# CederGroupHub/chgnet

Hardware: AMD Instinct MI355X
Metric: structures/s (energy+force+stress) on batched ~50-atom crystals (higher is better)
Workload: dtype f32; 1 GPU; 1024 x LiMnO2 5x1x1 (40 atoms, sigma=0.01 frac perturbation) per GPU, task efs; structures_per_gpu=1024, atoms=40960, directed_bonds=3535504, angles=4125764, bond_graph_nodes=213755, weights=random-init 0.3.0 architecture (tests/golden/weights_seed0.npz), parallelism=structures sharded over 1 GPU(s), RCCL all-gather of energies only, process_group_ranks=1, energies_in_all_gather=1024, comm=none (single rank)

## Files before the change

chgnet_amd/csrc/kernels_angle_w.h:

```cpp
#pragma once

#include "blk_shape.h"
#include "kernels_conv.h"

namespace chg {

constexpr int TS64 = D + PAD;
constexpr int TILE64_FLOATS = TILE_ROWS * TS64;
constexpr int WIN_LIST = 32;
constexpr int WIN_MAX_GRID = 1024;
constexpr int WIN_MIN_ATOMS_PER_WAVE = 3;

struct WinIndex {
  int* flag;
  int *wave_head, *next_atom;
  int* xatom;
  int *na, *boff, *aoff;
  int* toff;
  int* toff4;
  int *head, *rank;
  int* list;
  int *q_a, *q_ctr, *q_b1c, *q_b2c, *q_ab1, *q_ab2;
  int* abbond;
  int4* rows;
// ... 116 lines not shown
  }
  w.xatom[i] = lo;
}

__device__ __forceinline__ unsigned wave_min_u32(unsigned v) {
#define CHG_DPP_MIN(ctrl) v = min(v, (unsigned)__builtin_amdgcn_update_dpp((int)v, (int)v, (ctrl), 0xF, 0xF, false))
  CHG_DPP_MIN(0xB1);
  CHG_DPP_MIN(0x4E);
  CHG_DPP_MIN(0x141);
  CHG_DPP_MIN(0x140);
#undef CHG_DPP_MIN
  const auto r = __builtin_amdgcn_permlane16_swap(v, v, false, false);
  const unsigned s = min((unsigned)r[0], (unsigned)r[1]);
  const auto q = __builtin_amdgcn_permlane32_swap(s, s, false, false);
  return min((unsigned)q[0], (unsigned)q[1]);
}

static __global__ __launch_bounds__(64) void k_win_schedule(int grid, WinIndex w) {
  const int gi = blockIdx.x, lane = threadIdx.x;
  const int spx = grid >> 6;
  const int x = gi / spx, sub = gi - x * spx;
  const int head_slot = ((((sub << 3) + (lane / WAVES)) << 3) + x) * WAVES + (lane % WAVES);
  if (w.flag[0] != 1) { w.wave_head[head_slot] = -1; return; }
  const int c0 = w.xatom[gi], c1 = w.xatom[gi + 1];
  unsigned load = 0;
  int head = -1, tail = -1;
  for (int cb = c0; cb < c1; cb += 64) {
    const int nn = w.na[min(cb + lane, c1 - 1)];
    const int m = min(64, c1 - cb);
    for (int i = 0; i < m; ++i) {
      const int n = __builtin_amdgcn_readlane(nn, i);
      if (n < 2) continue;
      const unsigned cost = (unsigned)(n * (n - 1) + TILE_ROWS - 1) / TILE_ROWS + 1;
      const unsigned best = wave_min_u32((load << 6) | (unsigned)lane);
      if ((int)(best & 63u) == lane) {
        const int c = cb + i;
        load += cost;
        w.next_atom[c] = -1;
        if (tail < 0) head = c; else w.next_atom[tail] = c;
        tail = c;
      }
    }
  }
  w.wave_head[head_slot] = head;
}

static __global__ void k_win_atoms(int N, WinIndex w) {
  const int c = blockIdx.x * blockDim.x + threadIdx.x;
  if (c < N) w.atoms[c] = make_int4(w.na[c], w.aoff[c], w.boff[c], w.next_atom[c]);
}

struct AngleWArgs {
  AngleArgs a;
  WinIndex w;
  int n_atoms;
};

struct AngleBwdWArgs {
  const int* flag;
  const float* image;
  const float* w_ang;
  GatedW gw;
  const float *R, *S, *ang, *wbgc, *Gagg, *zsave;
  float *Gang, *GR, *GS, *Gwbgc;
  int first_gang;
  const int4* rows;
  const int* abbond;
  const int4* atoms;
  const int* wave_head;
  const int *toff, *na, *aoff, *boff, *q_a, *q_b1c, *q_b2c, *q_ab2;
  int n_atoms;
};
inline AngleBwdWArgs angle_bwd_w_args(const AngleArgs& a, const WinIndex& w, int n_atoms) {
  AngleBwdWArgs k{};
  k.flag = w.flag; k.image = a.image; k.w_ang = a.w_ang; k.gw = a.gw;
  k.R = a.R; k.S = a.S; k.ang = a.ang; k.wbgc = a.wbgc; k.Gagg = a.Gagg; k.zsave = a.zsave;
  k.Gang = a.Gang; k.GR = a.GR; k.GS = a.GS; k.Gwbgc = a.Gwbgc; k.first_gang = a.first_gang;
  k.rows = w.rows; k.abbond = w.abbond; k.atoms = w.atoms; k.wave_head = w.wave_head;
  k.toff = w.toff; k.na = w.na; k.aoff = w.aoff; k.boff = w.boff; k.q_a = w.q_a; k.q_b1c = w.q_b1c; k.q_b2c = w.q_b2c; k.q_ab2 = w.q_ab2;
  k.n_atoms = n_atoms;
  return k;
}

template <class T, bool A32 = false>
__device__ __forceinline__ T index_load(const T* __restrict__ base, int i) {
  if constexpr (A32) return *reinterpret_cast<const T*>(reinterpret_cast<const char*>(base) + (unsigned)i * (unsigned)sizeof(T));
  else return base[i];
}
__device__ __forceinline__ int4 index_load_uniform(const int4* base, int i) {
#if defined(__HIP_DEVICE_COMPILE__)
  typedef const int __attribute__((address_space(4))) * ConstInt;
  ConstInt q = (ConstInt)(unsigned long long)(base + i);
  return make_int4(q[0], q[1], q[2], q[3]);
#else
  return base[i];
#endif
}

template <bool HIDDEN> constexpr int win_ns() { return HIDDEN ? 13 : 14; }
template <bool HIDDEN> constexpr int win_pst() { return 2 * D; }
constexpr size_t WIN_RM_ANG = rm_image_bytes(2 * D, D), WIN_RM_W2 = rm_image_bytes(D, D);

template <bool HIDDEN>
constexpr size_t angle_w_lds() {
  const size_t weights = HIDDEN ? WIN_RM_ANG + 2 * WIN_RM_W2 : 16 * (size_t)(2 * IMG128);
  return weights + sizeof(float) * (VEC_SLOTS * D + WAVES * TILE64_FLOATS + WAVES * win_ns<HIDDEN>() * win_pst<HIDDEN>());
}

struct Gather64 { f32x4 a[TILE_ROWS / 4], b[TILE_ROWS / 4], c[TILE_ROWS / 4]; };
template <bool A32 = false>
__device__ __forceinline__ void gather64_issue(Gather64& gr, const float* __restrict__ t0, int i0, int ld0, const float* __restrict__ t1, int i1,
                                               int ld1, const float* __restrict__ t2, int i2, int ld2, int lane, int c0 = 0, int c1 = 0, int c2 = 0) {
  const int sub = lane >> 4, t = lane & 15;
  int r0[TILE_ROWS / 4], r1[TILE_ROWS / 4], r2[TILE_ROWS / 4];
#pragma unroll
  for (int it = 0; it < TILE_ROWS / 4; ++it) {
    const int rr = 4 * it + sub;
    r0[it] = __shfl(i0, rr); r1[it] = __shfl(i1, rr); r2[it] = __shfl(i2, rr);
  }
#pragma unroll
  for (int it = 0; it < TILE_ROWS / 4; ++it) {
    gr.a[it] = *grow<f32x4, A32>(t0, (unsigned)r0[it], ld0, c0 + 4 * t);
    gr.b[it] = *grow<f32x4, A32>(t1, (unsigned)r1[it], ld1, c1 + 4 * t);
    gr.c[it] = *grow<f32x4, A32>(t2, (unsigned)r2[it], ld2, c2 + 4 * t);
  }
}
__device__ __forceinline__ void gather64_commit(const Gather64& gr, float* tile, int lane) {
  const int sub = lane >> 4, t = lane & 15;
#pragma unroll
  for (int it = 0; it < TILE_ROWS / 4; ++it)
    *reinterpret_cast<f32x4*>(tile + (4 * it + sub) * TS64 + 4 * t) = (gr.a[it] + gr.b[it]) + gr.c[it];
}

struct Cols64 { float v[TILE_ROWS]; };
__device__ __forceinline__ void to_columns(const V64& x, float* T, float* Trow, int g, int lane, Cols64& c) {
  write_dl<VT>(Trow, g, x.t);
  __builtin_amdgcn_wave_barrier();
#pragma unroll
  for (int rr = 0; rr < TILE_ROWS; ++rr) c.v[rr] = T[rr * TS64 + lane];
  __builtin_amdgcn_wave_barrier();
}
__device__ __forceinline__ int fresh_uniform(int v) {
  asm volatile("" : "+s"(v));
  return v;
}
__device__ __forceinline__ unsigned run_starts64(int key, int cur, int nvalid, int lane) {
  const int prev = __builtin_amdgcn_update_dpp(cur, key, 0x111 , 0xF, 0xF, false);
  return (unsigned)__builtin_amdgcn_ballot_w64(key != prev && lane < nvalid);
}
template <int NB, bool A32 = false>
__device__ __forceinline__ void run_sum64(const Cols64 (&c)[NB], int nvalid, int key, unsigned starts, float (&sum)[NB], int& cur, float* __restrict__ dst,
                                          int ld, int col) {
  nvalid = fresh_uniform(nvalid);
#pragma unroll
  for (int rr = 0; rr < TILE_ROWS; ++rr) {
    if (rr < nvalid) {
      if (starts & (1u << rr)) {
        if (cur >= 0) {
          float* d = grow<float, A32>(dst, (unsigned)cur, ld, col);
#pragma unroll
          for (int q = 0; q < NB; ++q) atomicAdd(d + q * D, sum[q]);
        }
#pragma unroll
        for (int q = 0; q < NB; ++q) sum[q] = 0.f;
        cur = __builtin_amdgcn_readlane(key, rr);
      }
#pragma unroll
      for (int q = 0; q < NB; ++q) sum[q] += c[q].v[rr];
    }
  }
}
template <int NB, bool A32 = false>
__device__ __forceinline__ void run_flush64(float (&sum)[NB], int& cur, float* __restrict__ dst, int ld, int col) {
  if (cur >= 0) {
    float* d = grow<float, A32>(dst, (unsigned)cur, ld, col);
#pragma unroll
    for (int q = 0; q < NB; ++q) atomicAdd(d + q * D, sum[q]);
  }
#pragma unroll
  for (int q = 0; q < NB; ++q) sum[q] = 0.f;
  cur = -1;
}
template <bool A32 = false>
__device__ __forceinline__ void row_add64(const Cols64& c, int nvalid, float* __restrict__ base, int row, int ld, int lane) {
  nvalid = fresh_uniform(nvalid);
#pragma unroll
  for (int rr = 0; rr < TILE_ROWS; ++rr)
    if (rr < nvalid) atomicAdd(grow<float, A32>(base, (unsigned)__builtin_amdgcn_readlane(row, rr), ld, lane), c.v[rr]);
}
template <int NB>
__device__ __forceinline__ void private_add(const Cols64 (&c)[NB], int nvalid, int slot, float* pacc, float* dump, int lane) {
  nvalid = fresh_uniform(nvalid);
#pragma unroll
  for (int rr = 0; rr < TILE_ROWS; rr += 2) {
    const int sa = __builtin_amdgcn_readlane(slot, rr), sb = __builtin_amdgcn_readlane(slot, rr + 1);
    float* pa = (rr < nvalid && sa >= 0) ? pacc + sa * (NB * D) : dump;
    float* pb = (rr + 1 < nvalid && sb >= 0) ? pacc + sb * (NB * D) : dump + NB * D;
    float a[NB], b[NB];
#pragma unroll
    for (int q = 0; q < NB; ++q) { a[q] = pa[q * D + lane]; b[q] = pb[q * D + lane]; }
#pragma unroll
    for (int q = 0; q < NB; ++q) { pa[q * D + lane] = a[q] + c[q].v[rr]; pb[q * D + lane] = b[q] + c[q].v[rr + 1]; }
  }
}

template <bool HIDDEN, bool TEAM = false, bool ZS = false, bool A32 = false>
__global__ __launch_bounds__(BLOCK) CHG_TWO_WAVES void k_angle_bwd_w(AngleBwdWArgs pw) {
  const AngleBwdWArgs& p = pw;
  const AngleBwdWArgs& w = pw;
  if (w.flag[0] != 1) return;
  extern __shared__ __attribute__((aligned(16))) float smem[];
  constexpr int NS = win_ns<HIDDEN>(), PST = win_pst<HIDDEN>();
  constexpr int MODE = HIDDEN ? 2 : 1;
  float* Wang = smem;
  float* WangT = HIDDEN ? Wang : Wang + 4 * IMG128;
  float* W2c = HIDDEN ? Wang + WIN_RM_ANG / 4 : WangT + 4 * IMG128;
  float* W2g = W2c + (HIDDEN ? WIN_RM_W2 / 4 : 0);
  float* vecs = W2g + (HIDDEN ? WIN_RM_W2 / 4 : 0);
  float* tiles = vecs + VEC_SLOTS * D;
  float* paccs = tiles + WAVES * TILE64_FLOATS;
  const int tid = threadIdx.x, lane = tid & 63, j = lane & 15, g = lane >> 4;
  const int wave = __builtin_amdgcn_readfirstlane(tid >> 6);
  static_assert((size_t)AngleLds<HIDDEN, true>::tiles * sizeof(float) == (HIDDEN ? WIN_RM_ANG + 2 * WIN_RM_W2 : 16 * (size_t)(2 * IMG128)) + sizeof(float) * VEC_SLOTS * D,
                "the per-atom adjoints share the weight image of k_angle<HIDDEN, true>");
  if (p.image) {
    stage_image<AngleLds<HIDDEN, true>::tiles / 4, BLOCK>(smem, p.image, tid);
  } else if (HIDDEN) {
// ... 233 lines not shown
```

chgnet_amd/csrc/kernels_conv.h:

```cpp
#pragma once

#include "mfma_tile.h"
#include "mfma_split.h"

namespace chg {

constexpr int TS = 2 * D + PAD;
constexpr int WS = D + PAD;
constexpr int TILE_FLOATS = TILE_ROWS * TS;
constexpr int VEC_SLOTS = 6;
constexpr int IMG64 = 1024, IMG128 = 2048;
constexpr int angle_split(bool hidden, bool bwd) { return (hidden && bwd) ? 2 : 1; }

struct GatedW {
  const float *w2c, *b2c, *w2g, *b2g, *ln1_g, *ln1_b, *ln2_g, *ln2_b;
};

__device__ __forceinline__ void stage_gated_vecs(float* vecs, const GatedW& gw, bool hidden, int tid) {
  if (hidden) {
    stage_vector(vecs + 0 * D, gw.b2c, D, tid);
    stage_vector(vecs + 1 * D, gw.b2g, D, tid);
  }
  stage_vector(vecs + 2 * D, gw.ln1_g, D, tid);
  stage_vector(vecs + 3 * D, gw.ln1_b, D, tid);
// ... 474 lines not shown
    bn_n2 = bond_node(p, r1 >> 1);
  }
  stage_image<ac_fwd_image_floats() / 4, 64 * NW>(smem, p.image, tid);
  __syncthreads();
  for (int v = 0; v < ts.count; ++v) {
    const int row0 = ts.at(v) * tstride;
    const int nvalid = min(TILE_ROWS, p.n_edges - row0);
    const int c = c_nx;
    const bool node = bn_nx >= 0;
    const V64 wv = wv_nx;
    gather_commit_h(gr, T, TS, lane);
    __builtin_amdgcn_wave_barrier();
    V64 x;
    read_dl<VT>(Trow, g, x.t);
    __builtin_amdgcn_wave_barrier();
    gather_commit_p(gr, T, TS, lane);
    __builtin_amdgcn_wave_barrier();
    c_nx = c_n2; n_nx = n_n2; bn_nx = bn_n2;
    if (v + 1 < ts.count) {
      const int r1 = row_of(v + 1);
      gather_issue_ph<A32>(gr, p.P, c_nx, p.P + 2 * D, n_nx, 4 * D, 4 * D, p.hb0, bond_row_offset<A32>(p, r1 >> 1, bn_nx), lane);
      read_dl_g<VT, A32>(p.wag, (unsigned)(r1 >> 1), D, g, wv_nx.t);
      const int r2 = row_of(v + 2);
      c_n2 = p.e_center[r2]; n_n2 = p.e_nbr[r2];
      bn_n2 = bond_node(p, r2 >> 1);
    }
    f32x4 z[2 * VT];
    if (!node) {
      read_dl<2 * VT>(vecs + VEC_SLOTS * D, g, z);
    } else {
#pragma unroll
      for (int ft = 0; ft < 2 * VT; ++ft) z[ft] = f32x4{0.f, 0.f, 0.f, 0.f};
    }
    gemm_split<VT, 2 * VT, false, true>(z, Ib, 2 * D, x.t, j, g);
    if (p.Qout && !(j & 1) && j < nvalid) {
      write_dl_g<2 * VT, A32>(p.Qout, (unsigned)((row0 + j) >> 1), 2 * D, g, z);
    }
    {
      f32x4 ps[2 * VT];
      read_dl<2 * VT>(Trow, g, ps);
#pragma unroll
      for (int ft = 0; ft < 2 * VT; ++ft) z[ft] += ps[ft];
    }
    V64 zc{{z[0], z[1], z[2], z[3]}}, zg{{z[4], z[5], z[6], z[7]}};
    GatedState s;
    V64 y;
    gated_forward<true, false, false, 1, true>(zc, zg, W2c, W2g, vecs, j, g, s, y);
    gather_take(gr);
    asm volatile("" : "+v"(c_n2), "+v"(n_n2), "+v"(bn_n2));
    CHG_EV(ft) asm volatile("" : "+v"(wv_nx.t[ft]));
    __builtin_amdgcn_wave_barrier();
    V64 m;
    CHG_EV(ft) m.t[ft] = y.t[ft] * wv.t[ft];
    write_dl<VT>(Trow, g, m.t);
    __builtin_amdgcn_wave_barrier();
    {
      float acc1 = 0.f, acc2 = 0.f;
      int cur1 = __builtin_amdgcn_readlane(c, 0), cur2 = __builtin_amdgcn_readlane(c, 1);
#pragma unroll
      for (int b = 0; b < TILE_ROWS / 2; ++b) {
        if (2 * b < nvalid) {
          const int c1 = __builtin_amdgcn_readlane(c, 2 * b), c2 = __builtin_amdgcn_readlane(c, 2 * b + 1);
          if (c1 != cur1) {
            tile_atomic_add(grow<float, A32>(p.agg, (unsigned)cur1, D, lane), acc1);
            acc1 = 0.f;
            cur1 = c1;
          }
          if (c2 != cur2) {
            tile_atomic_add(grow<float, A32>(p.agg, (unsigned)cur2, D, lane), acc2);
            acc2 = 0.f;
            cur2 = c2;
          }
          acc1 += T[(2 * b) * TS + lane];
          acc2 += T[(2 * b + 1) * TS + lane];
        }
      }
      tile_atomic_add(grow<float, A32>(p.agg, (unsigned)cur1, D, lane), acc1);
      tile_atomic_add(grow<float, A32>(p.agg, (unsigned)cur2, D, lane), acc2);
    }
    __builtin_amdgcn_wave_barrier();
  }
}

template <bool STORE_GQ = true, bool A32 = false>
__device__ __forceinline__ void acbwd_scatter(const float* T, int c, int nvalid, int k0, const AtomConvArgs& p, int lane) {
  float a1[4] = {0.f, 0.f, 0.f, 0.f}, a2[4] = {0.f, 0.f, 0.f, 0.f};
  int cur1 = __builtin_amdgcn_readlane(c, 0), cur2 = __builtin_amdgcn_readlane(c, 1);
#pragma unroll
  for (int b = 0; b < TILE_ROWS / 2; ++b) {
    if (2 * b < nvalid) {
      const float e0 = T[(2 * b) * TS + lane], e1 = T[(2 * b) * TS + 64 + lane];
      const float o0 = T[(2 * b + 1) * TS + lane], o1 = T[(2 * b + 1) * TS + 64 + lane];
      if (STORE_GQ) {
        float* q = p.GQ + (size_t)(k0 + b) * 2 * D + lane;
        q[0] = e0 + o0;
        q[64] = e1 + o1;
      }
      const int c1 = __builtin_amdgcn_readlane(c, 2 * b), c2 = __builtin_amdgcn_readlane(c, 2 * b + 1);
      if (c1 != cur1) {
        float* d = grow<float, A32>(p.GP, (unsigned)cur1, 4 * D, lane);
        tile_atomic_add(d, a1[0]); tile_atomic_add(d + 64, a1[1]); tile_atomic_add(d + 128, a1[2]); tile_atomic_add(d + 192, a1[3]);
        a1[0] = a1[1] = a1[2] = a1[3] = 0.f;
        cur1 = c1;
      }
      if (c2 != cur2) {
        float* d = grow<float, A32>(p.GP, (unsigned)cur2, 4 * D, lane);
        tile_atomic_add(d, a2[0]); tile_atomic_add(d + 64, a2[1]); tile_atomic_add(d + 128, a2[2]); tile_atomic_add(d + 192, a2[3]);
        a2[0] = a2[1] = a2[2] = a2[3] = 0.f;
        cur2 = c2;
      }
      a1[0] += e0; a1[1] += e1; a1[2] += o0; a1[3] += o1;
      a2[0] += o0; a2[1] += o1; a2[2] += e0; a2[3] += e1;
    }
  }
  float* d1 = grow<float, A32>(p.GP, (unsigned)cur1, 4 * D, lane);
  tile_atomic_add(d1, a1[0]); tile_atomic_add(d1 + 64, a1[1]); tile_atomic_add(d1 + 128, a1[2]); tile_atomic_add(d1 + 192, a1[3]);
  float* d2 = grow<float, A32>(p.GP, (unsigned)cur2, 4 * D, lane);
  tile_atomic_add(d2, a2[0]); tile_atomic_add(d2 + 64, a2[1]); tile_atomic_add(d2 + 128, a2[2]); tile_atomic_add(d2 + 192, a2[3]);
}

template <bool TRAIN, bool A32 = false>
__global__ __launch_bounds__(BLOCK) CHG_TWO_WAVES void k_atomconv_bwd(AtomConvArgs p) {
  constexpr bool FUSE_GQ = !TRAIN;
  constexpr int NW = WAVES;
  constexpr bool RM = FUSE_GQ;
  extern __shared__ __attribute__((aligned(16))) float smem[];
  constexpr int HMODE = RM ? 2 : 1;
  float* vecs = RM ? smem + 2 * AC_RM_IMG : smem + 4 * 4 * IMG64;
  const h16x8* IbT = reinterpret_cast<const h16x8*>(vecs + VEC_SLOTS * D);
  float* tiles = vecs + VEC_SLOTS * D + (FUSE_GQ ? 4 * IMG128 : 0);
  const float* W2c = smem;
  const float* W2g = RM ? smem + AC_RM_IMG : smem + 4 * IMG64;
  const float* W2cT = RM ? W2c : smem + 2 * 4 * IMG64;
  const float* W2gT = RM ? W2g : smem + 3 * 4 * IMG64;
  const int tid = threadIdx.x, lane = tid & 63, j = lane & 15, g = lane >> 4;
  const int wave = __builtin_amdgcn_readfirstlane(tid >> 6);
  float* T = tiles + wave * TILE_FLOATS;
  float* Trow = T + j * TS;
  const int ntiles = (p.n_edges + TILE_ROWS - 1) / TILE_ROWS;
  const TileSeq ts = wave_tile_seq<!TRAIN>(ntiles, NW, wave);
  const int last_row = p.n_edges - 1;
  int c, n, k;
  {
    const int row = max(0, min(ts.at(0) * TILE_ROWS + j, last_row));
    c = p.e_center[row]; n = p.e_nbr[row]; k = row >> 1;
    GatherRegs gr;
    gather_issue128<A32>(gr, p.P, c, p.P + 2 * D, n, p.Q, k, 4 * D, 4 * D, 2 * D, lane);
    if (TRAIN) atomconv_bwd_stage(smem, p, tid, 64 * NW);
    else stage_image<ac_bwd_rm_image_floats() / 4, 64 * NW>(smem, p.image, tid);
    gather_commit128(gr, T, TS, lane);
  }
  __syncthreads();
  TrainTile tt{};
  tt.T = T; tt.lane = lane;
  for (int v = 0; v < ts.count; ++v) {
    const int row0 = ts.at(v) * TILE_ROWS;
    const int nvalid = min(TILE_ROWS, p.n_edges - row0);
    if (TRAIN) {
      tt.nvalid = nvalid;
      tt.hrow = j < nvalid ? p.dumpH + (size_t)(row0 + j) * 2 * D : nullptr;
      tt.grow = j < nvalid ? p.dumpG + (size_t)(row0 + j) * 2 * D : nullptr;
    }
    int cn, nn, kn;
    {
      const int row = max(0, min(ts.at(v + 1) * TILE_ROWS + j, last_row));
      cn = p.e_center[row]; nn = p.e_nbr[row]; kn = row >> 1;
    }
    V64 wv, gm;
    read_dl_g<VT, A32>(p.wag, (unsigned)k, D, g, wv.t);
    read_dl_g<VT, A32>(p.GA, (unsigned)c, D, g, gm.t);
    const int k0 = row0 >> 1, nb = nvalid >> 1;
    float* gwag_rows = grow<float, A32>(p.Gwag, (unsigned)k0, D, lane);
    float prev[TILE_ROWS / 2];
#pragma unroll
    for (int b = 0; b < TILE_ROWS / 2; ++b) prev[b] = p.first_wag ? 0.f : gwag_rows[(size_t)min(b, nb - 1) * D];
    __builtin_amdgcn_wave_barrier();
    V64 zc, zg;
    read_dl<VT>(Trow, g, zc.t);
    read_dl<VT>(Trow + D, g, zg.t);
    GatedState s;
    V64 y;
    gated_forward<true, false, TRAIN, HMODE>(zc, zg, W2c, W2g, vecs, j, g, s, y, &tt);
    asm volatile("" : "+v"(cn), "+v"(nn));
    V64 gy, gw, gzc, gzg;
    CHG_EV(ft) {
      gw.t[ft] = gm.t[ft] * y.t[ft];
      gy.t[ft] = gm.t[ft] * wv.t[ft];
    }
    __builtin_amdgcn_wave_barrier();
    write_dl<VT>(Trow, g, gw.t);
    __builtin_amdgcn_wave_barrier();
    {
      float* dst = gwag_rows;
#pragma unroll
      for (int b = 0; b < TILE_ROWS / 2; ++b) prev[b] += T[(2 * b) * TS + lane] + T[(2 * b + 1) * TS + lane];
      if (nvalid == TILE_ROWS) {
#pragma unroll
        for (int b = 0; b < TILE_ROWS / 2; ++b) dst[(size_t)b * D] = prev[b];
      } else {
#pragma unroll
        for (int b = 0; b < TILE_ROWS / 2; ++b)
          if (b < nb) dst[(size_t)b * D] = prev[b];
      }
    }
    gated_backward<true, false, TRAIN, HMODE>(gy, zc, zg, W2cT, W2gT, vecs, j, g, s, gzc, gzg, &tt);
    if (FUSE_GQ) {
      float* gb_row = grow<float, A32>(p.Gb, (unsigned)(k0 + (j >> 1)), D, 4 * g);
      const bool owner = !(j & 1) && j < nvalid;
      V64 old = zero64();
      if (p.gb_accumulate && owner) {
        CHG_EV(ft) old.t[ft] = *reinterpret_cast<const f32x4*>(gb_row + 16 * ft);
      }
      f32x4 gz[2 * VT] = {gzc.t[0], gzc.t[1], gzc.t[2], gzc.t[3], gzg.t[0], gzg.t[1], gzg.t[2], gzg.t[3]};
      V64 gq = zero64();
      gemm_split<2 * VT, VT, true>(gq.t, IbT, D, gz, j, g);
      CHG_EW(ft, r) gq.t[ft][r] += __shfl_xor(gq.t[ft][r], 1);
      CHG_EV(ft) gq.t[ft] += old.t[ft];
      CHG_EV(ft) asm volatile("" : "+v"(gq.t[ft]));
      if (owner) {
        CHG_EV(ft) *reinterpret_cast<f32x4*>(gb_row + 16 * ft) = gq.t[ft];
      }
    }
    __builtin_amdgcn_wave_barrier();
    write_dl<VT>(Trow, g, gzc.t);
    write_dl<VT>(Trow + D, g, gzg.t);
    __builtin_amdgcn_wave_barrier();
    if (v + 1 < ts.count) {
      GatherRegs gr;
      gather_issue128<A32>(gr, p.P, cn, p.P + 2 * D, nn, p.Q, kn, 4 * D, 4 * D, 2 * D, lane);
      acbwd_scatter<!FUSE_GQ, A32>(T, c, nvalid, k0, p, lane);
      __builtin_amdgcn_wave_barrier();
      gather_commit128(gr, T, TS, lane);
    } else {
      acbwd_scatter<!FUSE_GQ, A32>(T, c, nvalid, k0, p, lane);
    }
    c = cn; n = nn; k = kn;
  }
  if (TRAIN) {
#pragma unroll
    for (int q = 0; q < 4; ++q) atomicAdd(p.g_ln + q * D + lane, tt.ln[q]);
  }
}

struct AngleArgs {
  const float* R;
  const float* S;
  const float* ang;
  const float* wbgc;
  const int *a_ctr, *a_b1c, *a_b2c;
  int n_angles;
  const float* w_ang;
  GatedW gw;
  const float* image;
  int slot;
  float* out;
  const float* Gagg;
  float* Gang;
  float* GR;
  float* GS;
  float* Gwbgc;
  int first_gang;
  const int* skip_flag;
  float* zsave;
  float* dumpG;
  float* dumpH;
  float* dumpZ;
  float* g_ln;
};

template <bool HIDDEN, int NW = WAVES, bool BWD = false>
constexpr size_t angle_lds() {
  if (angle_split(HIDDEN, BWD) == 2) return rm_image_bytes(2 * D, D) + 2 * rm_image_bytes(D, D) + sizeof(float) * (VEC_SLOTS * D + NW * TILE_FLOATS);
  return 16 * (size_t)((BWD ? 2 : 1) * IMG128 + (HIDDEN ? 2 * IMG64 : 0)) + sizeof(float) * (VEC_SLOTS * D + NW * TILE_FLOATS);
}


template <bool HIDDEN, bool BWD>
struct AngleLds {
  static constexpr int SPLIT = angle_split(HIDDEN, BWD);
  static constexpr int wangT = SPLIT == 2 ? 0 : 4 * IMG128;
  static constexpr int w2c = SPLIT == 2 ? (int)(rm_image_bytes(2 * D, D) / 4) : wangT + (BWD ? 4 * IMG128 : 0);
  static constexpr int w2 = HIDDEN ? (SPLIT == 2 ? (int)(rm_image_bytes(D, D) / 4) : 4 * IMG64) : 0;
  static constexpr int w2g = w2c + w2;
  static constexpr int vecs = w2g + w2;
  static constexpr int tiles = vecs + VEC_SLOTS * D;
};
template <bool HIDDEN, bool BWD>
__device__ __forceinline__ void angle_stage(float* base, const float* __restrict__ w_ang, const GatedW& gw, int tid, int nthreads) {
  using L = AngleLds<HIDDEN, BWD>;
  float* Wang = base;
  float* WangT = base + L::wangT;
  float* W2c = base + L::w2c;
  float* W2g = base + L::w2g;
  if (L::SPLIT == 2) {
    stage_rm(reinterpret_cast<_Float16*>(Wang), w_ang, 2 * D, D, tid, nthreads);
    stage_rm(reinterpret_cast<_Float16*>(W2c), gw.w2c, D, D, tid, nthreads);
    stage_rm(reinterpret_cast<_Float16*>(W2g), gw.w2g, D, D, tid, nthreads);
  } else {
    stage_split<false>(reinterpret_cast<h16x8*>(Wang), w_ang, 2 * D, D, tid, nthreads);
    if (BWD) stage_split<true>(reinterpret_cast<h16x8*>(WangT), w_ang, 2 * D, D, tid, nthreads);
    if (HIDDEN) {
      stage_split<false>(reinterpret_cast<h16x8*>(W2c), gw.w2c, D, D, tid, nthreads);
      stage_split<false>(reinterpret_cast<h16x8*>(W2g), gw.w2g, D, D, tid, nthreads);
    }
  }
  stage_gated_vecs(base + L::vecs, gw, HIDDEN, tid);
}
template <bool HIDDEN, bool BWD>
__global__ __launch_bounds__(BLOCK) void k_angle_image(const float* w_ang, GatedW gw, float* out) {
  angle_stage<HIDDEN, BWD>(out, w_ang, gw, threadIdx.x, BLOCK);
}

template <bool HIDDEN, bool BWD, int NW = WAVES, bool TRAIN = false, bool A32 = false>
__global__ __launch_bounds__(64 * NW) CHG_TWO_WAVES void k_angle(AngleArgs p) {
  static_assert(!TRAIN || BWD, "TRAIN is a variant of the adjoint kernels");
  if (!TRAIN && p.skip_flag && *p.skip_flag == 1) return;
  extern __shared__ __attribute__((aligned(16))) float smem[];
  constexpr int SPLIT = angle_split(HIDDEN, BWD);
// ... 297 lines not shown
```

chgnet_amd/csrc/mfma_tile.h:

```cpp
#pragma once

#include <hip/hip_runtime.h>
#include <stdint.h>


namespace chg {

typedef float f32x4 __attribute__((ext_vector_type(4)));

constexpr int D = 64;
constexpr int TILE_ROWS = 16;
constexpr int WAVES = 8;
constexpr int BLOCK = 64 * WAVES;
constexpr int BLOCK_ROWS = TILE_ROWS * WAVES;
constexpr int PAD = 4;
constexpr int VT = 4;
constexpr float LN_EPS = 1e-5f;
constexpr int MFMA_R = 4;

struct V64 { f32x4 t[VT]; };

__device__ __forceinline__ int dfeat(int ft, int r, int g) { return 16 * ft + 4 * g + r; }

__device__ __forceinline__ f32x4 zero4() { return f32x4{0.f, 0.f, 0.f, 0.f}; }
__device__ __forceinline__ V64 zero64() { return V64{{zero4(), zero4(), zero4(), zero4()}}; }

__device__ __forceinline__ float sigmoidf_(float x) {
  return __builtin_amdgcn_rcpf(1.0f + __builtin_amdgcn_exp2f(-1.4426950408889634f * x));
}
__device__ __forceinline__ float siluf_(float x) { return x * sigmoidf_(x); }
__device__ __forceinline__ float dsiluf_(float x) {
  const float s = sigmoidf_(x);
  return s * (1.0f + x * (1.0f - s));
}

typedef float f32x2 __attribute__((ext_vector_type(2)));
__device__ __forceinline__ f32x2 sigmoid2(f32x2 x) {
  f32x2 t = x * -1.4426950408889634f;
  t[0] = __builtin_amdgcn_exp2f(t[0]); t[1] = __builtin_amdgcn_exp2f(t[1]);
  t = t + 1.0f;
  t[0] = __builtin_amdgcn_rcpf(t[0]); t[1] = __builtin_amdgcn_rcpf(t[1]);
  return t;
}
__device__ __forceinline__ f32x4 sigmoid4(f32x4 x) {
  const f32x2 lo = sigmoid2(f32x2{x[0], x[1]}), hi = sigmoid2(f32x2{x[2], x[3]});
  return f32x4{lo[0], lo[1], hi[0], hi[1]};
}
__device__ __forceinline__ float hsum4(f32x4 v) { return (v[0] + v[1]) + (v[2] + v[3]); }
#define CHG_EV(ft) _Pragma("unroll") for (int ft = 0; ft < VT; ++ft)

#define CHG_EW(ft, r) _Pragma("unroll") for (int ft = 0; ft < VT; ++ft) _Pragma("unroll") for (int r = 0; r < 4; ++r)

template <class T, bool A32 = false>
__device__ __forceinline__ const T* grow(const float* __restrict__ base, unsigned r, int ld, int c) {
  if constexpr (A32) return reinterpret_cast<const T*>(reinterpret_cast<const char*>(base) + (r * (unsigned)(4 * ld) + (unsigned)(4 * c)));
  else return reinterpret_cast<const T*>(base + (size_t)r * ld + c);
}
template <class T, bool A32 = false>
__device__ __forceinline__ T* grow(float* __restrict__ base, unsigned r, int ld, int c) {
  if constexpr (A32) return reinterpret_cast<T*>(reinterpret_cast<char*>(base) + (r * (unsigned)(4 * ld) + (unsigned)(4 * c)));
  else return reinterpret_cast<T*>(base + (size_t)r * ld + c);
}
template <int NT>
__device__ __forceinline__ void read_dl(const float* row, int g, f32x4 (&x)[NT]) {
#pragma unroll
  for (int ft = 0; ft < NT; ++ft) x[ft] = *reinterpret_cast<const f32x4*>(row + 16 * ft + 4 * g);
}
template <int NT>
__device__ __forceinline__ void write_dl(float* row, int g, const f32x4 (&x)[NT]) {
#pragma unroll
  for (int ft = 0; ft < NT; ++ft) *reinterpret_cast<f32x4*>(row + 16 * ft + 4 * g) = x[ft];
}

template <int NT, bool A32 = false>
__device__ __forceinline__ void read_dl_g(const float* __restrict__ base, unsigned r, int ld, int g, f32x4 (&x)[NT]) {
#pragma unroll
  for (int ft = 0; ft < NT; ++ft) x[ft] = *grow<f32x4, A32>(base, r, ld, 16 * ft + 4 * g);
}
template <int NT, bool A32 = false>
__device__ __forceinline__ void write_dl_g(float* __restrict__ base, unsigned r, int ld, int g, const f32x4 (&x)[NT]) {
#pragma unroll
  for (int ft = 0; ft < NT; ++ft) *grow<f32x4, A32>(base, r, ld, 16 * ft + 4 * g) = x[ft];
}

template <int NT, bool A32 = false>
__device__ __forceinline__ void read_dl_g_nt(const float* __restrict__ base, unsigned r, int ld, int g, f32x4 (&x)[NT]) {
#pragma unroll
  for (int ft = 0; ft < NT; ++ft) x[ft] = __builtin_nontemporal_load(grow<f32x4, A32>(base, r, ld, 16 * ft + 4 * g));
}
template <int NT, bool A32 = false>
__device__ __forceinline__ void write_dl_g_nt(float* __restrict__ base, unsigned r, int ld, int g, const f32x4 (&x)[NT]) {
#pragma unroll
  for (int ft = 0; ft < NT; ++ft) __builtin_nontemporal_store(x[ft], grow<f32x4, A32>(base, r, ld, 16 * ft + 4 * g));
}

template <int KT, int NFT>
__device__ __forceinline__ void gemm_dl(f32x4 (&acc)[NFT], const float* W, int ws, const f32x4 (&x)[KT], int i, int g) {
  const float* wbase = W + i * ws + 4 * g;
#pragma unroll
  for (int kt = 0; kt < KT; ++kt) {
    f32x4 w[NFT];
#pragma unroll
    for (int fo = 0; fo < NFT; ++fo) w[fo] = *reinterpret_cast<const f32x4*>(wbase + 16 * fo * ws + 16 * kt);
#pragma unroll
    for (int r = 0; r < MFMA_R; ++r)
#pragma unroll
      for (int fo = 0; fo < NFT; ++fo) acc[fo] = __builtin_amdgcn_mfma_f32_16x16x4f32(w[fo][r], x[kt][r], acc[fo], 0, 0, 0);
  }
}

template <int NFT>
__device__ __forceinline__ void gemm_t_load(float (&a)[4][NFT], const float* W, int ws, int kt, int i, int g) {
#pragma unroll
  for (int r = 0; r < 4; ++r) {
    const float* wrow = W + dfeat(kt, r, g) * ws + i;
#pragma unroll
    for (int fo = 0; fo < NFT; ++fo) a[r][fo] = wrow[16 * fo];
  }
}
template <int NFT>
__device__ __forceinline__ void gemm_t_touch(float (&a)[4][NFT]) {
#pragma unroll
  for (int r = 0; r < 4; ++r)
#pragma unroll
    for (int fo = 0; fo < NFT; ++fo) asm volatile("" : "+v"(a[r][fo]));
}
template <int KT, int NFT>
__device__ __forceinline__ void gemm_dl_t(f32x4 (&acc)[NFT], const float* W, int ws, const f32x4 (&x)[KT], int i, int g) {
  float a[2][4][NFT];
  gemm_t_load<NFT>(a[0], W, ws, 0, i, g);
#pragma unroll
  for (int kt = 0; kt < KT; ++kt) {
    if (kt + 1 < KT) gemm_t_load<NFT>(a[(kt + 1) & 1], W, ws, kt + 1, i, g);
    gemm_t_touch<NFT>(a[kt & 1]);
#pragma unroll
    for (int r = 0; r < MFMA_R; ++r)
#pragma unroll
      for (int fo = 0; fo < NFT; ++fo) acc[fo] = __builtin_amdgcn_mfma_f32_16x16x4f32(a[kt & 1][r][fo], x[kt][r], acc[fo], 0, 0, 0);
  }
}

__device__ __forceinline__ float quad_sum(float v) {
  const unsigned u = __float_as_uint(v);
  const auto r = __builtin_amdgcn_permlane16_swap(u, u, false, false);
// ... 115 lines not shown
  float acc[NC];
#pragma unroll
  for (int c = 0; c < NC; ++c) acc[c] = 0.f;
  int cur = __builtin_amdgcn_readlane(key, 0);
#pragma unroll
  for (int rr = 0; rr < TILE_ROWS; ++rr) {
    const int kk = __builtin_amdgcn_readlane(key, rr);
    if (kk != cur) {
      if (cur >= 0) {
#pragma unroll
        for (int c = 0; c < NC; ++c) tile_atomic_add(grow<float, A32>(dst, (unsigned)cur, ldd, 64 * c + lane), acc[c]);
      }
#pragma unroll
      for (int c = 0; c < NC; ++c) acc[c] = 0.f;
      cur = kk;
    }
#pragma unroll
    for (int c = 0; c < NC; ++c) acc[c] += tile[rr * stride + 64 * c + lane];
  }
  if (cur >= 0) {
#pragma unroll
    for (int c = 0; c < NC; ++c) tile_atomic_add(grow<float, A32>(dst, (unsigned)cur, ldd, 64 * c + lane), acc[c]);
  }
}

template <int W, bool A32 = false>
__device__ __forceinline__ void row_atomic_add(const float* tile, int stride, int key, int nvalid, float* __restrict__ dst,
                                               int ldd, int lane) {
#pragma unroll
  for (int rr = 0; rr < TILE_ROWS; ++rr) {
    const int kk = __builtin_amdgcn_readlane(key, rr);
    if (kk >= 0) {
#pragma unroll
      for (int c = 0; c < W / 64; ++c) tile_atomic_add(grow<float, A32>(dst, (unsigned)kk, ldd, 64 * c + lane), tile[rr * stride + 64 * c + lane]);
    }
  }
}

template <bool A32 = false>
__device__ __forceinline__ void gather_sum128(float* tile, int stride, const float* __restrict__ t0, int i0,
                                              const float* __restrict__ t1, int i1, const float* __restrict__ t2, int i2,
                                              int ld0, int ld1, int ld2, int lane) {
  const int hw = lane >> 5, t = lane & 31;
  int r0[TILE_ROWS / 2], r1[TILE_ROWS / 2], r2[TILE_ROWS / 2];
#pragma unroll
  for (int it = 0; it < TILE_ROWS / 2; ++it) {
    const int rr = 2 * it + hw;
    r0[it] = __shfl(i0, rr); r1[it] = __shfl(i1, rr); r2[it] = __shfl(i2, rr);
  }
  f32x4 a[TILE_ROWS / 2], b[TILE_ROWS / 2], c[TILE_ROWS / 2];
#pragma unroll
  for (int it = 0; it < TILE_ROWS / 2; ++it) {
    a[it] = *grow<f32x4, A32>(t0, (unsigned)r0[it], ld0, 4 * t);
    b[it] = *grow<f32x4, A32>(t1, (unsigned)r1[it], ld1, 4 * t);
    c[it] = *grow<f32x4, A32>(t2, (unsigned)r2[it], ld2, 4 * t);
  }
#pragma unroll
  for (int it = 0; it < TILE_ROWS / 2; ++it) {
    const int rr = 2 * it + hw;
    *reinterpret_cast<f32x4*>(tile + rr * stride + 4 * t) = (a[it] + b[it]) + c[it];
  }
}

struct GatherRegs { f32x4 a[TILE_ROWS / 2], b[TILE_ROWS / 2], c[TILE_ROWS / 2]; };
__device__ __forceinline__ void gather_take(GatherRegs& gr);

template <bool A32 = false>
__device__ __forceinline__ void gather_issue128(GatherRegs& gr, const float* __restrict__ t0, int i0, const float* __restrict__ t1,
                                                int i1, const float* __restrict__ t2, int i2, int ld0, int ld1, int ld2, int lane) {
  const int hw = lane >> 5, t = lane & 31;
  int r0[TILE_ROWS / 2], r1[TILE_ROWS / 2], r2[TILE_ROWS / 2];
#pragma unroll
  for (int it = 0; it < TILE_ROWS / 2; ++it) {
    const int rr = 2 * it + hw;
    r0[it] = __shfl(i0, rr); r1[it] = __shfl(i1, rr); r2[it] = __shfl(i2, rr);
  }
#pragma unroll
  for (int it = 0; it < TILE_ROWS / 2; ++it) {
    gr.a[it] = *grow<f32x4, A32>(t0, (unsigned)r0[it], ld0, 4 * t);
    gr.b[it] = *grow<f32x4, A32>(t1, (unsigned)r1[it], ld1, 4 * t);
    gr.c[it] = *grow<f32x4, A32>(t2, (unsigned)r2[it], ld2, 4 * t);
  }
}
__device__ __forceinline__ void gather_commit128(const GatherRegs& gr, float* tile, int stride, int lane) {
  const int hw = lane >> 5, t = lane & 31;
#pragma unroll
  for (int it = 0; it < TILE_ROWS / 2; ++it)
    *reinterpret_cast<f32x4*>(tile + (2 * it + hw) * stride + 4 * t) = (gr.a[it] + gr.b[it]) + gr.c[it];
}

struct GatherPH { f32x4 a[TILE_ROWS / 2], b[TILE_ROWS / 2], h[TILE_ROWS / 4]; };
__device__ __forceinline__ void gather_take(GatherPH& gr) {
#pragma unroll
  for (int it = 0; it < TILE_ROWS / 2; ++it) asm volatile("" : "+v"(gr.a[it]), "+v"(gr.b[it]));
#pragma unroll
  for (int it = 0; it < TILE_ROWS / 4; ++it) asm volatile("" : "+v"(gr.h[it]));
}
__device__ __forceinline__ void gather_take(GatherRegs& gr) {
#pragma unroll
  for (int it = 0; it < TILE_ROWS / 2; ++it) asm volatile("" : "+v"(gr.a[it]), "+v"(gr.b[it]), "+v"(gr.c[it]));
}
template <bool A32 = false>
__device__ __forceinline__ void gather_issue_ph(GatherPH& gr, const float* __restrict__ t0, int i0, const float* __restrict__ t1, int i1, int ld0,
                                                int ld1, const float* __restrict__ hbase, long hoff, int lane) {
  const int hw = lane >> 5, t = lane & 31, sub = lane >> 4, t16 = lane & 15;
  int r0[TILE_ROWS / 2], r1[TILE_ROWS / 2];
  long ho[TILE_ROWS / 4];
#pragma unroll
  for (int it = 0; it < TILE_ROWS / 2; ++it) {
    const int rr = 2 * it + hw;
    r0[it] = __shfl(i0, rr); r1[it] = __shfl(i1, rr);
  }
  const int hlo = (int)(hoff & 0xffffffffL), hhi = (int)(hoff >> 32);
#pragma unroll
  for (int it = 0; it < TILE_ROWS / 4; ++it) {
    const int rr = 4 * it + sub;
    if constexpr (A32) ho[it] = (long)(unsigned)__shfl(hlo, rr);
    else ho[it] = ((long)__shfl(hhi, rr) << 32) | (unsigned)__shfl(hlo, rr);
  }
#pragma unroll
  for (int it = 0; it < TILE_ROWS / 2; ++it) {
    gr.a[it] = *grow<f32x4, A32>(t0, (unsigned)r0[it], ld0, 4 * t);
    gr.b[it] = *grow<f32x4, A32>(t1, (unsigned)r1[it], ld1, 4 * t);
  }
#pragma unroll
  for (int it = 0; it < TILE_ROWS / 4; ++it) {
    if constexpr (A32) gr.h[it] = *reinterpret_cast<const f32x4*>(reinterpret_cast<const char*>(hbase) + (4u * (unsigned)ho[it] + 16u * (unsigned)t16));
    else gr.h[it] = *reinterpret_cast<const f32x4*>(hbase + ho[it] + 4 * t16);
  }
}
__device__ __forceinline__ void gather_commit_p(const GatherPH& gr, float* tile, int stride, int lane) {
  const int hw = lane >> 5, t = lane & 31;
#pragma unroll
  for (int it = 0; it < TILE_ROWS / 2; ++it) *reinterpret_cast<f32x4*>(tile + (2 * it + hw) * stride + 4 * t) = gr.a[it] + gr.b[it];
}
__device__ __forceinline__ void gather_commit_h(const GatherPH& gr, float* tile, int stride, int lane) {
  const int sub = lane >> 4, t = lane & 15;
#pragma unroll
  for (int it = 0; it < TILE_ROWS / 4; ++it) *reinterpret_cast<f32x4*>(tile + (4 * it + sub) * stride + 4 * t) = gr.h[it];
}

struct Rows64 { f32x4 v[TILE_ROWS / 4]; };
template <bool A32 = false>
__device__ __forceinline__ void rows64_issue(Rows64& rr, const float* __restrict__ src, int idx, int lane) {
  const int sub = lane >> 4, t = lane & 15;
  int r[TILE_ROWS / 4];
#pragma unroll
  for (int it = 0; it < TILE_ROWS / 4; ++it) r[it] = __shfl(idx, 4 * it + sub);
#pragma unroll
  for (int it = 0; it < TILE_ROWS / 4; ++it) rr.v[it] = *grow<f32x4, A32>(src, (unsigned)r[it], D, 4 * t);
}
__device__ __forceinline__ void rows64_commit(const Rows64& rr, float* tile, int stride, int lane) {
  const int sub = lane >> 4, t = lane & 15;
#pragma unroll
  for (int it = 0; it < TILE_ROWS / 4; ++it) *reinterpret_cast<f32x4*>(tile + (4 * it + sub) * stride + 4 * t) = rr.v[it];
}
template <bool OPAQUE = false, bool A32 = false>
__device__ __forceinline__ void scatter_rows64_add(const float* tile, int stride, float* __restrict__ dst, int idx, int nvalid, int lane,
                                                   const Rows64& old) {
  const int sub = lane >> 4, t = lane & 15;
  f32x4 v[TILE_ROWS / 4];
  int r[TILE_ROWS / 4];
#pragma unroll
  for (int it = 0; it < TILE_ROWS / 4; ++it) {
    const int rr = 4 * it + sub;
    r[it] = __shfl(idx, rr);
// ... 49 lines not shown
```

Baseline: 40650 structures/s.

## Restructure atom-conv backward scatter to overlap next-tile gathers with scatter

The atom-conv backward loop now issues the next tile's Q-row gather before the FUSE_GQ GEMM and the P-row gathers right after it. The gradient tile is read into registers and committed before the Gb store and the atomic scatter, so the global loads overlap more compute. The scatter computes segment starts once with a DPP compare plus ballot instead of readlane comparisons per row, and masks invalid rows up front. Index loads and the Gwag prefetch also use 32-bit addressing and uniform paths. The cost is more live registers (GatherRegs, AcGz), which could lower occupancy or cause spills.

After: 40960 structures/s (median of 6 runs). Within noise of the previous version (+0.7%).

```diff
diff --git a/chgnet_amd/csrc/kernels_angle_w.h b/chgnet_amd/csrc/kernels_angle_w.h
--- a/chgnet_amd/csrc/kernels_angle_w.h
+++ b/chgnet_amd/csrc/kernels_angle_w.h
@@ -222,11 +222,6 @@
   return k;
 }
 
-template <class T, bool A32 = false>
-__device__ __forceinline__ T index_load(const T* __restrict__ base, int i) {
-  if constexpr (A32) return *reinterpret_cast<const T*>(reinterpret_cast<const char*>(base) + (unsigned)i * (unsigned)sizeof(T));
-  else return base[i];
-}
 __device__ __forceinline__ int4 index_load_uniform(const int4* base, int i) {
 #if defined(__HIP_DEVICE_COMPILE__)
   typedef const int __attribute__((address_space(4))) * ConstInt;
@@ -279,10 +274,6 @@
 #pragma unroll
   for (int rr = 0; rr < TILE_ROWS; ++rr) c.v[rr] = T[rr * TS64 + lane];
   __builtin_amdgcn_wave_barrier();
-}
-__device__ __forceinline__ int fresh_uniform(int v) {
-  asm volatile("" : "+s"(v));
-  return v;
 }
 __device__ __forceinline__ unsigned run_starts64(int key, int cur, int nvalid, int lane) {
   const int prev = __builtin_amdgcn_update_dpp(cur, key, 0x111 , 0xF, 0xF, false);
diff --git a/chgnet_amd/csrc/kernels_conv.h b/chgnet_amd/csrc/kernels_conv.h
--- a/chgnet_amd/csrc/kernels_conv.h
+++ b/chgnet_amd/csrc/kernels_conv.h
@@ -580,41 +580,68 @@
   }
 }
 
+struct AcGz { float e0[TILE_ROWS / 2], e1[TILE_ROWS / 2], o0[TILE_ROWS / 2], o1[TILE_ROWS / 2]; };
+__device__ __forceinline__ unsigned pair_run_starts(int c, int nvalid, int lane) {
+  const int prev = __builtin_amdgcn_update_dpp(c, c, 0x112 , 0xF, 0xF, false);
+  return (unsigned)__builtin_amdgcn_ballot_w64(c != prev && lane < nvalid);
+}
+__device__ __forceinline__ void acbwd_read_gz(const float* T, int nvalid, int lane, AcGz& z) {
+#pragma unroll
+  for (int b = 0; b < TILE_ROWS / 2; ++b) {
+    z.e0[b] = T[(2 * b) * TS + lane]; z.e1[b] = T[(2 * b) * TS + 64 + lane];
+    z.o0[b] = T[(2 * b + 1) * TS + lane]; z.o1[b] = T[(2 * b + 1) * TS + 64 + lane];
+  }
+  if (nvalid < TILE_ROWS) {
+    const int nv = fresh_uniform(nvalid);
+#pragma unroll
+    for (int b = 1; b < TILE_ROWS / 2; ++b)
+      if (2 * b >= nv) z.e0[b] = z.e1[b] = z.o0[b] = z.o1[b] = 0.f;
+  }
+}
+template <bool A32 = false>
+__device__ __forceinline__ void acbwd_flush(float* __restrict__ GP, int atom, const float (&a)[4], int lane) {
+  float* d = grow<float, A32>(GP, (unsigned)atom, 4 * D, lane);
+  tile_atomic_add(d, a[0]); tile_atomic_add(d + 64, a[1]); tile_atomic_add(d + 128, a[2]); tile_atomic_add(d + 192, a[3]);
+}
+template <bool STORE_GQ = true, bool A32 = false>
+__device__ __forceinline__ void acbwd_scatter(const AcGz& z, unsigned starts, int c, int nvalid, int k0, const AtomConvArgs& p, int lane) {
+  if (STORE_GQ) {
+    const int nb = fresh_uniform(nvalid) >> 1;
+#pragma unroll
+    for (int b = 0; b < TILE_ROWS / 2; ++b) {
+      if (b < nb) {
+        float* q = p.GQ + (size_t)(k0 + b) * 2 * D + lane;
+        q[0] = z.e0[b] + z.o0[b];
+        q[64] = z.e1[b] + z.o1[b];
+      }
+    }
+  }
+  float a1[4] = {z.e0[0], z.e1[0], z.o0[0], z.o1[0]}, a2[4] = {z.o0[0], z.o1[0], z.e0[0], z.e1[0]};
+  int cur1 = __builtin_amdgcn_readlane(c, 0), cur2 = __builtin_amdgcn_readlane(c, 1);
+#pragma unroll
+  for (int b = 1; b < TILE_ROWS / 2; ++b) {
+    if (starts & (1u << (2 * b))) {
+      acbwd_flush<A32>(p.GP, cur1, a1, lane);
+      a1[0] = a1[1] = a1[2] = a1[3] = 0.f;
+      cur1 = __builtin_amdgcn_readlane(c, 2 * b);
+    }
+    if (starts & (2u << (2 * b))) {
+      acbwd_flush<A32>(p.GP, cur2, a2, lane);
+      a2[0] = a2[1] = a2[2] = a2[3] = 0.f;
+      cur2 = __builtin_amdgcn_readlane(c, 2 * b + 1);
+    }
+    a1[0] += z.e0[b]; a1[1] += z.e1[b]; a1[2] += z.o0[b]; a1[3] += z.o1[b];
+    a2[0] += z.o0[b]; a2[1] += z.o1[b]; a2[2] += z.e0[b]; a2[3] += z.e1[b];
+  }
+  acbwd_flush<A32>(p.GP, cur1, a1, lane);
+  acbwd_flush<A32>(p.GP, cur2, a2, lane);
+}
 template <bool STORE_GQ = true, bool A32 = false>
 __device__ __forceinline__ void acbwd_scatter(const float* T, int c, int nvalid, int k0, const AtomConvArgs& p, int lane) {
-  float a1[4] = {0.f, 0.f, 0.f, 0.f}, a2[4] = {0.f, 0.f, 0.f, 0.f};
-  int cur1 = __builtin_amdgcn_readlane(c, 0), cur2 = __builtin_amdgcn_readlane(c, 1);
-#pragma unroll
-  for (int b = 0; b < TILE_ROWS / 2; ++b) {
-    if (2 * b < nvalid) {
-      const float e0 = T[(2 * b) * TS + lane], e1 = T[(2 * b) * TS + 64 + lane];
-      const float o0 = T[(2 * b + 1) * TS + lane], o1 = T[(2 * b + 1) * TS + 64 + lane];
-      if (STORE_GQ) {
-        float* q = p.GQ + (size_t)(k0 + b) * 2 * D + lane;
-        q[0] = e0 + o0;
-        q[64] = e1 + o1;
-      }
-      const int c1 = __builtin_amdgcn_readlane(c, 2 * b), c2 = __builtin_amdgcn_readlane(c, 2 * b + 1);
-      if (c1 != cur1) {
-        float* d = grow<float, A32>(p.GP, (unsigned)cur1, 4 * D, lane);
-        tile_atomic_add(d, a1[0]); tile_atomic_add(d + 64, a1[1]); tile_atomic_add(d + 128, a1[2]); tile_atomic_add(d + 192, a1[3]);
-        a1[0] = a1[1] = a1[2] = a1[3] = 0.f;
-        cur1 = c1;
-      }
-      if (c2 != cur2) {
-        float* d = grow<float, A32>(p.GP, (unsigned)cur2, 4 * D, lane);
-        tile_atomic_add(d, a2[0]); tile_atomic_add(d + 64, a2[1]); tile_atomic_add(d + 128, a2[2]); tile_atomic_add(d + 192, a2[3]);
-        a2[0] = a2[1] = a2[2] = a2[3] = 0.f;
-        cur2 = c2;
-      }
-      a1[0] += e0; a1[1] += e1; a1[2] += o0; a1[3] += o1;
-      a2[0] += o0; a2[1] += o1; a2[2] += e0; a2[3] += e1;
-    }
-  }
-  float* d1 = grow<float, A32>(p.GP, (unsigned)cur1, 4 * D, lane);
-  tile_atomic_add(d1, a1[0]); tile_atomic_add(d1 + 64, a1[1]); tile_atomic_add(d1 + 128, a1[2]); tile_atomic_add(d1 + 192, a1[3]);
-  float* d2 = grow<float, A32>(p.GP, (unsigned)cur2, 4 * D, lane);
-  tile_atomic_add(d2, a2[0]); tile_atomic_add(d2 + 64, a2[1]); tile_atomic_add(d2 + 128, a2[2]); tile_atomic_add(d2 + 192, a2[3]);
+  nvalid = __builtin_amdgcn_readfirstlane(nvalid);
+  AcGz z;
+  acbwd_read_gz(T, nvalid, lane, z);
+  acbwd_scatter<STORE_GQ, A32>(z, pair_run_starts(c, nvalid, lane), c, nvalid, k0, p, lane);
 }
 
 template <bool TRAIN, bool A32 = false>
@@ -641,7 +668,7 @@
   int c, n, k;
   {
     const int row = max(0, min(ts.at(0) * TILE_ROWS + j, last_row));
-    c = p.e_center[row]; n = p.e_nbr[row]; k = row >> 1;
+    c = index_load<int, A32>(p.e_center, row); n = index_load<int, A32>(p.e_nbr, row); k = row >> 1;
     GatherRegs gr;
     gather_issue128<A32>(gr, p.P, c, p.P + 2 * D, n, p.Q, k, 4 * D, 4 * D, 2 * D, lane);
     if (TRAIN) atomconv_bwd_stage(smem, p, tid, 64 * NW);
@@ -662,7 +689,7 @@
     int cn, nn, kn;
     {
       const int row = max(0, min(ts.at(v + 1) * TILE_ROWS + j, last_row));
-      cn = p.e_center[row]; nn = p.e_nbr[row]; kn = row >> 1;
+      cn = index_load<int, A32>(p.e_center, row); nn = index_load<int, A32>(p.e_nbr, row); kn = row >> 1;
     }
     V64 wv, gm;
     read_dl_g<VT, A32>(p.wag, (unsigned)k, D, g, wv.t);
@@ -670,8 +697,17 @@
     const int k0 = row0 >> 1, nb = nvalid >> 1;
     float* gwag_rows = grow<float, A32>(p.Gwag, (unsigned)k0, D, lane);
     float prev[TILE_ROWS / 2];
-#pragma unroll
-    for (int b = 0; b < TILE_ROWS / 2; ++b) prev[b] = p.first_wag ? 0.f : gwag_rows[(size_t)min(b, nb - 1) * D];
+    if (p.first_wag) {
+#pragma unroll
+      for (int b = 0; b < TILE_ROWS / 2; ++b) prev[b] = 0.f;
+    } else if (nvalid == TILE_ROWS) {
+#pragma unroll
+      for (int b = 0; b < TILE_ROWS / 2; ++b) prev[b] = gwag_rows[b * D];
+    } else {
+      const int nbu = fresh_uniform(nb);
+#pragma unroll
+      for (int b = 0; b < TILE_ROWS / 2; ++b) prev[b] = *grow<float, A32>(p.Gwag, (unsigned)(k0 + min(b, nbu - 1)), D, lane);
+    }
     __builtin_amdgcn_wave_barrier();
     V64 zc, zg;
     read_dl<VT>(Trow, g, zc.t);
@@ -694,44 +730,51 @@
       for (int b = 0; b < TILE_ROWS / 2; ++b) prev[b] += T[(2 * b) * TS + lane] + T[(2 * b + 1) * TS + lane];
       if (nvalid == TILE_ROWS) {
 #pragma unroll
-        for (int b = 0; b < TILE_ROWS / 2; ++b) dst[(size_t)b * D] = prev[b];
+        for (int b = 0; b < TILE_ROWS / 2; ++b) dst[b * D] = prev[b];
       } else {
+        const int nbu = fresh_uniform(nb);
 #pragma unroll
         for (int b = 0; b < TILE_ROWS / 2; ++b)
-          if (b < nb) dst[(size_t)b * D] = prev[b];
+          if (b < nbu) dst[b * D] = prev[b];
       }
     }
     gated_backward<true, false, TRAIN, HMODE>(gy, zc, zg, W2cT, W2gT, vecs, j, g, s, gzc, gzg, &tt);
+    GatherRegs gr;
+    const bool more = v + 1 < ts.count;
+    gather_issue128_c<A32>(gr, p.Q, kn, 2 * D, lane);
+    V64 gq = zero64();
+    float* gb_row = nullptr;
+    const bool owner = !(j & 1) && j < nvalid;
     if (FUSE_GQ) {
-      float* gb_row = grow<float, A32>(p.Gb, (unsigned)(k0 + (j >> 1)), D, 4 * g);
-      const bool owner = !(j & 1) && j < nvalid;
+      gb_row = grow<float, A32>(p.Gb, (unsigned)(k0 + (j >> 1)), D, 4 * g);
       V64 old = zero64();
       if (p.gb_accumulate && owner) {
         CHG_EV(ft) old.t[ft] = *reinterpret_cast<const f32x4*>(gb_row + 16 * ft);
       }
       f32x4 gz[2 * VT] = {gzc.t[0], gzc.t[1], gzc.t[2], gzc.t[3], gzg.t[0], gzg.t[1], gzg.t[2], gzg.t[3]};
-      V64 gq = zero64();
       gemm_split<2 * VT, VT, true>(gq.t, IbT, D, gz, j, g);
       CHG_EW(ft, r) gq.t[ft][r] += __shfl_xor(gq.t[ft][r], 1);
       CHG_EV(ft) gq.t[ft] += old.t[ft];
+    }
+    gather_issue128_ab<A32>(gr, p.P, cn, p.P + 2 * D, nn, 4 * D, 4 * D, lane);
+    __builtin_amdgcn_wave_barrier();
+    write_dl<VT>(Trow, g, gzc.t);
+    write_dl<VT>(Trow + D, g, gzg.t);
+    __builtin_amdgcn_wave_barrier();
+    const unsigned starts = pair_run_starts(c, nvalid, lane);
+    AcGz z;
+    acbwd_read_gz(T, nvalid, lane, z);
+    if (more) {
+      __builtin_amdgcn_wave_barrier();
+      gather_commit128(gr, T, TS, lane);
+    }
+    if (FUSE_GQ) {
       CHG_EV(ft) asm volatile("" : "+v"(gq.t[ft]));
       if (owner) {
         CHG_EV(ft) *reinterpret_cast<f32x4*>(gb_row + 16 * ft) = gq.t[ft];
       }
     }
-    __builtin_amdgcn_wave_barrier();
-    write_dl<VT>(Trow, g, gzc.t);
-    write_dl<VT>(Trow + D, g, gzg.t);
-    __builtin_amdgcn_wave_barrier();
-    if (v + 1 < ts.count) {
-      GatherRegs gr;
-      gather_issue128<A32>(gr, p.P, cn, p.P + 2 * D, nn, p.Q, kn, 4 * D, 4 * D, 2 * D, lane);
-      acbwd_scatter<!FUSE_GQ, A32>(T, c, nvalid, k0, p, lane);
-      __builtin_amdgcn_wave_barrier();
-      gather_commit128(gr, T, TS, lane);
-    } else {
-      acbwd_scatter<!FUSE_GQ, A32>(T, c, nvalid, k0, p, lane);
-    }
+    acbwd_scatter<!FUSE_GQ, A32>(z, starts, c, nvalid, k0, p, lane);
     c = cn; n = nn; k = kn;
   }
   if (TRAIN) {
diff --git a/chgnet_amd/csrc/mfma_tile.h b/chgnet_amd/csrc/mfma_tile.h
--- a/chgnet_amd/csrc/mfma_tile.h
+++ b/chgnet_amd/csrc/mfma_tile.h
@@ -60,6 +60,15 @@
 __device__ __forceinline__ T* grow(float* __restrict__ base, unsigned r, int ld, int c) {
   if constexpr (A32) return reinterpret_cast<T*>(reinterpret_cast<char*>(base) + (r * (unsigned)(4 * ld) + (unsigned)(4 * c)));
   else return reinterpret_cast<T*>(base + (size_t)r * ld + c);
+}
+template <class T, bool A32 = false>
+__device__ __forceinline__ T index_load(const T* __restrict__ base, int i) {
+  if constexpr (A32) return *reinterpret_cast<const T*>(reinterpret_cast<const char*>(base) + (unsigned)i * (unsigned)sizeof(T));
+  else return base[i];
+}
+__device__ __forceinline__ int fresh_uniform(int v) {
+  asm volatile("" : "+s"(v));
+  return v;
 }
 template <int NT>
 __device__ __forceinline__ void read_dl(const float* row, int g, f32x4 (&x)[NT]) {
@@ -341,6 +350,28 @@
     gr.c[it] = *grow<f32x4, A32>(t2, (unsigned)r2[it], ld2, 4 * t);
   }
 }
+template <bool A32 = false>
+__device__ __forceinline__ void gather_issue128_c(GatherRegs& gr, const float* __restrict__ t2, int i2, int ld2, int lane) {
+  const int hw = lane >> 5, t = lane & 31;
+#pragma unroll
+  for (int it = 0; it < TILE_ROWS / 2; ++it) gr.c[it] = *grow<f32x4, A32>(t2, (unsigned)__shfl(i2, 2 * it + hw), ld2, 4 * t);
+}
+template <bool A32 = false>
+__device__ __forceinline__ void gather_issue128_ab(GatherRegs& gr, const float* __restrict__ t0, int i0, const float* __restrict__ t1, int i1,
+                                                   int ld0, int ld1, int lane) {
+  const int hw = lane >> 5, t = lane & 31;
+  int r0[TILE_ROWS / 2], r1[TILE_ROWS / 2];
+#pragma unroll
+  for (int it = 0; it < TILE_ROWS / 2; ++it) {
+    const int rr = 2 * it + hw;
+    r0[it] = __shfl(i0, rr); r1[it] = __shfl(i1, rr);
+  }
+#pragma unroll
+  for (int it = 0; it < TILE_ROWS / 2; ++it) {
+    gr.a[it] = *grow<f32x4, A32>(t0, (unsigned)r0[it], ld0, 4 * t);
+    gr.b[it] = *grow<f32x4, A32>(t1, (unsigned)r1[it], ld1, 4 * t);
+  }
+}
 __device__ __forceinline__ void gather_commit128(const GatherRegs& gr, float* tile, int stride, int lane) {
   const int hw = lane >> 5, t = lane & 31;
 #pragma unroll
```
